# LordLiang/DrawingSpinUp

Measured on NVIDIA H100. Metric: stylized frames/sec @512x512 (stage1+stage2), higher is better.
Workload: dtype fp16x3 (split fp16 hi+lo operands, fp32 accumulate)

## Files before the change

drawingspinup_b200/csrc/conv_wgmma.cu:

```cuda
#include "conv_device.cuh"

namespace dsu {

namespace {

__host__ __device__ inline uint32_t acc_pitch(int cout) { return static_cast<uint32_t>(cout) + 4; }

__host__ __device__ inline uint32_t par_bytes(int cout) { return (7 * cout + 4) * 4; }

__host__ __device__ inline int ric_halo_rows(int up) { return (kTileH >> up) + 2; }
__host__ __device__ inline int ric_halo_cols(int up) { return (kTileW >> up) + 2; }
constexpr uint32_t kStenBytes = kTileM * 8 * 8;

__host__ __device__ constexpr int halo_rows(int cout) { return cout <= 64 ? 16 : 8; }

constexpr int kRicRegMaxCout = 128;

__host__ __device__ constexpr bool register_a(ConvMode mode, int cout) {
    return mode == ConvMode::Halo || (mode == ConvMode::RicHalo && cout <= kRicRegMaxCout);
}

__host__ __device__ constexpr int ric_ctas_per_sm(ConvMode mode, int cout) {
    return mode == ConvMode::RicHalo && cout <= 64 ? 2 : 1;
}

struct SmemLayout {
    uint32_t stage_bytes;
    uint32_t halo;
    uint32_t halo_bytes;
    uint32_t aux;
    uint32_t par;
    uint32_t total;
};

__host__ __device__ inline SmemLayout smem_layout(ConvMode mode, int cout, int ksize, int up) {
    const bool halo = mode == ConvMode::Halo, ric_halo = mode == ConvMode::RicHalo;
    const int rows = halo ? halo_rows(cout) : kTileH;
    SmemLayout L;
    L.stage_bytes = (register_a(mode, cout) ? 0u : static_cast<uint32_t>(kABytes)) + static_cast<uint32_t>(cout) * 128u;
    L.halo = kStages * L.stage_bytes;
    L.halo_bytes = halo       ? static_cast<uint32_t>((rows + ksize - 1) * (kTileW + ksize - 1)) * 128u
                   : ric_halo ? static_cast<uint32_t>(ric_halo_rows(up) * ric_halo_cols(up)) * 128u : 0u;
    L.aux = L.halo + 2 * L.halo_bytes;
    const uint32_t main_end = L.aux + (halo ? 16u : ric_halo ? kStenBytes : 0u);
    const uint32_t staged = static_cast<uint32_t>(rows * kTileW) * acc_pitch(cout) * 4u;
    L.par = ((main_end > staged ? main_end : staged) + 15u) & ~15u;
    L.total = L.par + par_bytes(cout);
    return L;
}

__device__ __forceinline__ constexpr int ric_r0(int m) { return (m >= 2 && m <= 5) ? 0 : 1; }
__device__ __forceinline__ constexpr int ric_c0(int m) { return (m >= 4) ? 0 : 1; }

__device__ __forceinline__ void produce_tap(const ConvParams& p, int q, uint32_t a, int tid, int n, int ty0, int tx0) {
    const int j = tid & 7;
    const int prow = tid >> 3;
    const Slot sl = p.slots[q * 8 + j];
    const Seg sg = p.seg[sl.seg];
    const __half* sbase = sg.ptr + sl.choff;
    const uint32_t dst0 = a + static_cast<uint32_t>(prow) * 128u + (static_cast<uint32_t>(j ^ (prow & 7)) << 4);
    const size_t frame_in = static_cast<size_t>(n) * p.Hin * p.Win;
    const int ox = tx0 + (prow & 15), oy0 = ty0 + (prow >> 4);
    const int vx = ox * p.stride + sl.dx;
    const bool okx = sl.valid && static_cast<unsigned>(vx) < static_cast<unsigned>(p.Wv);
#pragma unroll
    for (int i = 0; i < 4; ++i) {
        const int vy = (oy0 + 2 * i) * p.stride + sl.dy;
        const bool ok = okx && static_cast<unsigned>(vy) < static_cast<unsigned>(p.Hv);
        const size_t pix = frame_in + static_cast<size_t>(vy >> p.up) * p.Win + (vx >> p.up);
        cp_async16(dst0 + i * 4096u, ok ? sbase + pix * sg.pitch : sbase, ok ? 16u : 0u);
    }
}

template <bool kExact>
struct RicItems {
    static constexpr int kSlots = kExact ? 4 : 8, kRowsPer = kExact ? 2 : 4, kRowStep = kTileM / kRowsPer;
};

struct RicWeightsH { __half2 w00, w01, w10, w11; };
struct RicWeightsF { float w0, w1, w2, w3; };

__device__ __forceinline__ __half2 h2_of(uint32_t v) { return *reinterpret_cast<const __half2*>(&v); }

__device__ __forceinline__ RicWeightsH ric_weights(uint2 wv) {
    const __half2 wa = h2_of(wv.x), wb = h2_of(wv.y);
    return {__low2half2(wa), __high2half2(wa), __low2half2(wb), __high2half2(wb)};
}
__device__ __forceinline__ RicWeightsF ric_weights(float2 l) {
    const float hy = 1.0f - l.x, hx = 1.0f - l.y;
    return {__fmul_rn(hy, hx), __fmul_rn(hy, l.y), __fmul_rn(l.x, hx), __fmul_rn(l.x, l.y)};
}
__device__ __forceinline__ uint32_t ric_blend(const RicWeightsH& w, uint32_t n00, uint32_t n01, uint32_t n10, uint32_t n11) {
    const __half2 o = __hfma2(w.w11, h2_of(n11), __hfma2(w.w10, h2_of(n10), __hfma2(w.w01, h2_of(n01), __hmul2(w.w00, h2_of(n00)))));
    return *reinterpret_cast<const uint32_t*>(&o);
}
__device__ __forceinline__ float ric_blend(const RicWeightsF& w, float v00, float v01, float v10, float v11) {
    return __fmaf_rn(w.w3, v11, __fmaf_rn(w.w2, v10, __fmaf_rn(w.w1, v01, __fmul_rn(w.w0, v00))));
}

template <bool kExact, typename Entry, typename Fetch>
__device__ __forceinline__ void ric_item(bool centre, const Entry& entry, const Fetch& fetch, uint32_t row, int d, uint32_t swz) {
    if constexpr (!kExact) {
        uint4 out;
        if (centre) {
            out = fetch(0, 0, 0);
        } else {
            const RicWeightsH w = ric_weights(entry());
            const uint4 n00 = fetch(0, 0, 0), n01 = fetch(0, 1, 0), n10 = fetch(1, 0, 0), n11 = fetch(1, 1, 0);
            out = make_uint4(ric_blend(w, n00.x, n01.x, n10.x, n11.x), ric_blend(w, n00.y, n01.y, n10.y, n11.y),
                             ric_blend(w, n00.z, n01.z, n10.z, n11.z), ric_blend(w, n00.w, n01.w, n10.w, n11.w));
        }
        st_shared_v4(row + ((static_cast<uint32_t>(d) ^ swz) << 4), out);
    } else {
        auto load8 = [&](int cy, int cx, float* v) {
            const uint4 lo = fetch(cy, cx, 0), hi = fetch(cy, cx, 1);
            v[0] = __uint_as_float(lo.x); v[1] = __uint_as_float(lo.y); v[2] = __uint_as_float(lo.z); v[3] = __uint_as_float(lo.w);
            v[4] = __uint_as_float(hi.x); v[5] = __uint_as_float(hi.y); v[6] = __uint_as_float(hi.z); v[7] = __uint_as_float(hi.w);
        };
        float f[8];
        if (centre) {
            load8(0, 0, f);
        } else {
            const RicWeightsF w = ric_weights(entry());
            float v00[8], v01[8], v10[8], v11[8];
            load8(0, 0, v00); load8(0, 1, v01); load8(1, 0, v10); load8(1, 1, v11);
#pragma unroll
            for (int c = 0; c < 8; ++c) f[c] = ric_blend(w, v00[c], v01[c], v10[c], v11[c]);
        }
        uint4 hi, lo;
        split8(f, hi, lo);
        st_shared_v4(row + ((static_cast<uint32_t>(d) ^ swz) << 4), hi);
        st_shared_v4(row + ((static_cast<uint32_t>(d + 4) ^ swz) << 4), lo);
    }
}

template <bool kExact>
__device__ __forceinline__ void produce_ric(const ConvParams& p, int q, uint32_t a, int tid, int n, int ty0, int tx0) {
    using It = RicItems<kExact>;
    const int blk = q / 9, t = q - 9 * blk;
    const int kq = t < 4 ? t : t - 1;
    const size_t frame_in = static_cast<size_t>(n) * p.Hin * p.Win;
    const int d = tid % It::kSlots, prow = tid / It::kSlots;
    const Slot sl = p.slots[blk * 8 + d];
    const Seg sg = p.seg[sl.seg];
    constexpr size_t kEsz = kExact ? sizeof(float) : sizeof(__half);
    const uint8_t* src = reinterpret_cast<const uint8_t*>(sg.ptr) + sl.choff * kEsz;
    const size_t pitch = static_cast<size_t>(sg.pitch) * kEsz;
#pragma unroll
    for (int i = 0; i < It::kRowsPer; ++i) {
        const int r = prow + It::kRowStep * i;
        const int oy = ty0 + (r >> 4), ox = tx0 + (r & 15);
        const bool live = sl.valid && oy < p.Hout && ox < p.Wout;
        const size_t e = live ? static_cast<size_t>(oy) * p.Wout + ox : 0;
        int dy0 = 0, dx0 = 0, m = 0;
        if (t != 4) {
            m = (kq + __ldg(p.ric_oct + e)) & 7;
            dy0 = ric_r0(m) - 1; dx0 = ric_c0(m) - 1;
        }
        auto fetch = [&](int cy, int cx, int h) {
            const int vy = oy + dy0 + cy, vx = ox + dx0 + cx;
            const bool ok = live && static_cast<unsigned>(vy) < static_cast<unsigned>(p.Hv) && static_cast<unsigned>(vx) < static_cast<unsigned>(p.Wv);
            const size_t pix = ok ? frame_in + static_cast<size_t>(vy >> p.up) * p.Win + (vx >> p.up) : 0;
            return ldg128_if(src + pix * pitch + 16 * h, ok);
        };
        auto entry = [&]() {
            if constexpr (kExact) return live ? __ldg(p.ric_lyx + e * 8 + m) : make_float2(0.0f, 0.0f);
            else return live ? __ldg(p.ric_wh + e * 8 + m) : make_uint2(0u, 0u);
        };
        ric_item<kExact>(t == 4, entry, fetch, a + static_cast<uint32_t>(r) * 128u, d, static_cast<uint32_t>(r & 7));
    }
}

struct RicTile {
    uint32_t halo, halo_bytes;
    uint32_t sten;
    uint32_t oct;
};

template <bool kExact>
__device__ __forceinline__ void stage_ric_stencil(const ConvParams& p, uint32_t sten, int tid, int ty0, int tx0) {
    const uint8_t* table = kExact ? reinterpret_cast<const uint8_t*>(p.ric_lyx) : reinterpret_cast<const uint8_t*>(p.ric_wh);
    for (int i = tid; i < kTileM * 8; i += kThreads) {
        const int r = i >> 3, m = i & 7;
        const int oy = ty0 + (r >> 4), ox = tx0 + (r & 15);
        const bool ok = oy < p.Hout && ox < p.Wout;
        const size_t e = ok ? static_cast<size_t>(oy) * p.Wout + ox : 0;
        cp_async8(sten + static_cast<uint32_t>(m * kTileM + r) * 8u, table + (e * 8 + m) * 8, ok ? 8u : 0u);
    }
}

__device__ __forceinline__ uint32_t ric_oct(const ConvParams& p, int r, int ty0, int tx0) {
    const int oy = ty0 + (r >> 4), ox = tx0 + (r & 15);
    return (oy < p.Hout && ox < p.Wout) ? static_cast<uint32_t>(__ldg(p.ric_oct + static_cast<size_t>(oy) * p.Wout + ox)) : 0u;
}

template <bool kExact>
__device__ __forceinline__ uint32_t load_ric_stencil(const ConvParams& p, uint32_t sten, int tid, int ty0, int tx0) {
    using It = RicItems<kExact>;
    stage_ric_stencil<kExact>(p, sten, tid, ty0, tx0);
    uint32_t oct = 0;
#pragma unroll
    for (int i = 0; i < It::kRowsPer; ++i) oct |= ric_oct(p, tid / It::kSlots + It::kRowStep * i, ty0, tx0) << (8 * i);
    return oct;
}

template <bool kExact>
__device__ __forceinline__ void load_ric_halo(const ConvParams& p, int blk, uint32_t halo, int tid, int n, int ty0, int tx0) {
    const int hw = ric_halo_cols(p.up), npix = ric_halo_rows(p.up) * hw;
    const int y0 = (ty0 >> p.up) - 1, x0 = (tx0 >> p.up) - 1;
    const int s = tid & 7;
    const Slot sl = p.slots[blk * 8 + (kExact ? s >> 1 : s)];
    const Seg sg = p.seg[sl.seg];
    constexpr size_t kEsz = kExact ? sizeof(float) : sizeof(__half);
    const uint8_t* sbase = reinterpret_cast<const uint8_t*>(sg.ptr) + (sl.choff + (kExact ? 4 * (s & 1) : 0)) * kEsz;
    const size_t pitch = static_cast<size_t>(sg.pitch) * kEsz;
    const size_t frame_in = static_cast<size_t>(n) * p.Hin * p.Win;
    for (int pix = tid >> 3; pix < npix; pix += kThreads / 8) {
        const int hy = pix / hw, hx = pix - hy * hw;
        const int y = y0 + hy, x = x0 + hx;
        const bool ok = sl.valid && static_cast<unsigned>(y) < static_cast<unsigned>(p.Hin) && static_cast<unsigned>(x) < static_cast<unsigned>(p.Win);
        const uint8_t* src = ok ? sbase + (frame_in + static_cast<size_t>(y) * p.Win + x) * pitch : sbase;
        cp_async16(halo + static_cast<uint32_t>(pix) * 128u + (static_cast<uint32_t>(s ^ (pix & 7)) << 4), src, ok ? 16u : 0u);
    }
}

template <bool kExact>
__device__ __forceinline__ void produce_ric_halo(const ConvParams& p, int q, uint32_t a, int tid, int ty0, int tx0, const RicTile& rt) {
    using It = RicItems<kExact>;
    const int blk = q / 9, t = q - 9 * blk;
    const int kq = t < 4 ? t : t - 1;
    const int d = tid % It::kSlots, prow = tid / It::kSlots;
    const bool valid = p.slots[blk * 8 + d].valid;
    const uint32_t halo = rt.halo + static_cast<uint32_t>(blk & 1) * rt.halo_bytes;
    const int hw = ric_halo_cols(p.up), y0 = (ty0 >> p.up) - 1, x0 = (tx0 >> p.up) - 1;
#pragma unroll
    for (int i = 0; i < It::kRowsPer; ++i) {
        const int r = prow + It::kRowStep * i;
        const int oy = ty0 + (r >> 4), ox = tx0 + (r & 15);
        const bool live = valid && oy < p.Hout && ox < p.Wout;
        int dy0 = 0, dx0 = 0, m = 0;
        if (t != 4) {
            m = (kq + (rt.oct >> (8 * i))) & 7;
            dy0 = ric_r0(m) - 1; dx0 = ric_c0(m) - 1;
        }
        auto fetch = [&](int cy, int cx, int h) {
            const int hp = (((oy + dy0 + cy) >> p.up) - y0) * hw + ((ox + dx0 + cx) >> p.up) - x0;
            const uint32_t s = kExact ? static_cast<uint32_t>(2 * d + h) : static_cast<uint32_t>(d);
            const uint4 v = ld_shared_v4(halo + static_cast<uint32_t>(hp) * 128u + ((s ^ static_cast<uint32_t>(hp & 7)) << 4));
            return live ? v : make_uint4(0u, 0u, 0u, 0u);
        };
        auto entry = [&]() {
            const uint2 raw = ld_shared_v2(rt.sten + static_cast<uint32_t>(m * kTileM + r) * 8u);
            if constexpr (kExact) return make_float2(__uint_as_float(raw.x), __uint_as_float(raw.y));
            else return raw;
        };
        ric_item<kExact>(t == 4, entry, fetch, a + static_cast<uint32_t>(r) * 128u, d, static_cast<uint32_t>(r & 7));
    }
}

struct RicLane {
    int r;
    int oy, ox;
    uint32_t live;
    uint32_t oct;
    int ax;
    int aslot;
};

__device__ __forceinline__ RicLane ric_lane(const ConvParams& p, int tid, int ty0, int tx0) {
    const int wg = tid >> 7, w = (tid >> 5) & 3, l = tid & 31;
    RicLane ln;
    ln.r = 64 * wg + 16 * w + (l >> 2);
    ln.oy = ty0 + (ln.r >> 4);
    ln.ox = tx0 + (ln.r & 15);
    ln.live = (ln.oy < p.Hout && ln.ox < p.Wout ? 1u : 0u) | (ln.oy < p.Hout && ln.ox + 8 < p.Wout ? 2u : 0u);
    const int ra = (ln.r & ~15) + (l & 7) + 8 * ((l >> 3) & 1);
    ln.ax = tx0 + (ra & 15);
    ln.aslot = l >> 4;
    ln.oct = ric_oct(p, ln.r, ty0, tx0) | ric_oct(p, ln.r + 8, ty0, tx0) << 8 | ric_oct(p, ra, ty0, tx0) << 16;
    return ln;
}

template <bool kExact>
__device__ __forceinline__ void build_ric_a(const ConvParams& p, int q, uint32_t halo, uint32_t sten, const RicLane& ln,
                                            int lane, int ty0, int tx0, uint32_t (*a)[4]) {
    const int t = q % 9, kq = t < 4 ? t : t - 1;
    const int hw = ric_halo_cols(p.up), y0 = (ty0 >> p.up) - 1, x0 = (tx0 >> p.up) - 1;
    auto hpix = [&](int vy, int vx) { return ((vy >> p.up) - y0) * hw + (vx >> p.up) - x0; };
    auto sector = [&](int j, int& dy0, int& dx0) {
        const int m = (kq + (ln.oct >> (8 * j))) & 7;
        dy0 = ric_r0(m) - 1; dx0 = ric_c0(m) - 1;
        return m;
    };
    if constexpr (!kExact) {
        auto slot = [&](int hp, int k) { return halo + static_cast<uint32_t>(hp) * 128u + ((static_cast<uint32_t>(2 * k + ln.aslot) ^ static_cast<uint32_t>(hp & 7)) << 4); };
        if (t == 4) {
            const int hp = hpix(ln.oy, ln.ax);
#pragma unroll
            for (int k = 0; k < 4; ++k) ldsm_x4(a[k], slot(hp, k));
        } else {
            int dy0, dx0;
            sector(2, dy0, dx0);
            const int vy = ln.oy + dy0, vx = ln.ax + dx0;
            const int h00 = hpix(vy, vx), h01 = hpix(vy, vx + 1), h10 = hpix(vy + 1, vx), h11 = hpix(vy + 1, vx + 1);
            RicWeightsH w[2];
#pragma unroll
            for (int j = 0; j < 2; ++j) w[j] = ric_weights(ld_shared_v2(sten + static_cast<uint32_t>(sector(j, dy0, dx0) * kTileM + ln.r + 8 * j) * 8u));
#pragma unroll
            for (int k = 0; k < 4; ++k) {
                uint32_t n00[4], n01[4], n10[4], n11[4];
                ldsm_x4(n00, slot(h00, k)); ldsm_x4(n01, slot(h01, k)); ldsm_x4(n10, slot(h10, k)); ldsm_x4(n11, slot(h11, k));
#pragma unroll
                for (int i = 0; i < 4; ++i) a[k][i] = ric_blend(w[i & 1], n00[i], n01[i], n10[i], n11[i]);
            }
        }
#pragma unroll
        for (int k = 0; k < 4; ++k)
#pragma unroll
            for (int i = 0; i < 4; ++i)
                if (!((ln.live >> (i & 1)) & 1)) a[k][i] = 0u;
    } else {
        const uint32_t th = static_cast<uint32_t>((lane & 3) >> 1), tb = static_cast<uint32_t>(lane & 1) * 8u;
        auto ld = [&](int hp, int g) {
            const uint32_t s = 2u * g + th;
            const uint2 v = ld_shared_v2(halo + static_cast<uint32_t>(hp) * 128u + ((s ^ static_cast<uint32_t>(hp & 7)) << 4) + tb);
            return make_float2(__uint_as_float(v.x), __uint_as_float(v.y));
        };
        auto put = [&](int j, int g, float2 f) {
            if (!((ln.live >> j) & 1)) f = make_float2(0.0f, 0.0f);
            uint32_t hi, lo;
            split2(f.x, f.y, hi, lo);
            a[g >> 1][j + 2 * (g & 1)] = hi;
            a[2 + (g >> 1)][j + 2 * (g & 1)] = lo;
        };
        if (t == 4) {
            float2 v[2][4];
#pragma unroll
            for (int j = 0; j < 2; ++j) {
                const int hp = hpix(ln.oy, ln.ox + 8 * j);
#pragma unroll
                for (int g = 0; g < 4; ++g) v[j][g] = ld(hp, g);
            }
#pragma unroll
            for (int j = 0; j < 2; ++j)
#pragma unroll
                for (int g = 0; g < 4; ++g) put(j, g, v[j][g]);
        } else {
#pragma unroll
            for (int j = 0; j < 2; ++j) {
                int dy0, dx0;
                const uint2 raw = ld_shared_v2(sten + static_cast<uint32_t>(sector(j, dy0, dx0) * kTileM + ln.r + 8 * j) * 8u);
                const int vy = ln.oy + dy0, vx = ln.ox + 8 * j + dx0;
                const int h00 = hpix(vy, vx), h01 = hpix(vy, vx + 1), h10 = hpix(vy + 1, vx), h11 = hpix(vy + 1, vx + 1);
                float2 v00[4], v01[4], v10[4], v11[4];
#pragma unroll
                for (int g = 0; g < 4; ++g) { v00[g] = ld(h00, g); v01[g] = ld(h01, g); v10[g] = ld(h10, g); v11[g] = ld(h11, g); }
                const RicWeightsF w = ric_weights(make_float2(__uint_as_float(raw.x), __uint_as_float(raw.y)));
#pragma unroll
                for (int g = 0; g < 4; ++g)
                    put(j, g, make_float2(ric_blend(w, v00[g].x, v01[g].x, v10[g].x, v11[g].x),
                                          ric_blend(w, v00[g].y, v01[g].y, v10[g].y, v11[g].y)));
            }
        }
    }
}

__device__ __forceinline__ void produce_b(const ConvParams& p, int q, uint32_t dst, int tid) {
    const uint8_t* src = p.wpack + static_cast<size_t>(q) * p.b_bytes;
    for (int i = tid; i < p.b_bytes / 16; i += kThreads) cp_async16(dst + 16u * i, src + 16 * i, 16u);
}

template <ConvMode kMode, bool kExact>
__device__ __forceinline__ void produce(const ConvParams& p, int q, uint32_t stage, int tid, int n, int ty0, int tx0, const RicTile& rt) {
    if constexpr (kMode == ConvMode::Tap) {
        produce_tap(p, q, stage, tid, n, ty0, tx0);
    } else if constexpr (kMode == ConvMode::Ric) {
        produce_ric<kExact>(p, q, stage, tid, n, ty0, tx0);
    } else {
        const int blk = q / 9;
        if (q == 9 * blk && blk + 1 < p.nblocks)
            load_ric_halo<kExact>(p, blk + 1, rt.halo + static_cast<uint32_t>((blk + 1) & 1) * rt.halo_bytes, tid, n, ty0, tx0);
        produce_ric_halo<kExact>(p, q, stage, tid, ty0, tx0, rt);
    }
    produce_b(p, q, stage + kABytes, tid);
}

template <int NC, int PN>
__device__ __forceinline__ void mma_chunk(float* acc, uint64_t da, uint64_t db, uint32_t km, uint32_t km2) {
    constexpr uint64_t kPieceStep = PN * 128 / 16;
    auto step = [&](int ka, int kb) {
#pragma unroll
        for (int j = 0; j < NC / PN; ++j) Wgmma<PN>::mma(acc + j * (PN / 2), da + 2 * ka, db + 2 * kb + j * kPieceStep);
    };
    if (km2) {
#pragma unroll
        for (int k = 0; k < 4; ++k)
            if ((km >> k) & 1) step(k, k & 1);
#pragma unroll
        for (int k = 0; k < 2; ++k)
            if ((km2 >> k) & 1) step(k, 2 + k);
    } else {
#pragma unroll
        for (int k = 0; k < 4; ++k)
            if ((km >> k) & 1) step(k, k);
    }
}

template <int NC, int PN, int MB, bool kExact>
__device__ __forceinline__ void mma_chunk_rs(float (*acc)[NC / 2], const uint32_t (*a)[4][4], uint64_t db) {
    constexpr uint64_t kPieceStep = PN * 128 / 16;
    auto step = [&](int ka, int kb) {
#pragma unroll
        for (int mb = 0; mb < MB; ++mb)
#pragma unroll
            for (int j = 0; j < NC / PN; ++j) Wgmma<PN>::mma_rs(acc[mb] + j * (PN / 2), a[mb][ka], db + 2 * kb + j * kPieceStep);
    };
#pragma unroll
    for (int k = 0; k < 4; ++k) step(k, kExact ? (k & 1) : k);
    if constexpr (kExact) {
#pragma unroll
        for (int k = 0; k < 2; ++k) step(k, 2 + k);
    }
}

template <int kRows>
__device__ __forceinline__ void load_halo(const ConvParams& p, int blk, uint32_t halo, int tid, int n, int ty0, int tx0) {
    const int hw = kTileW + p.ksize - 1, npix = (kRows + p.ksize - 1) * hw;
    const int s = tid & 7;
    const Slot sl = p.hslots[blk * 8 + s];
    const Seg sg = p.seg[sl.seg];
    const __half* sbase = sg.ptr + sl.choff;
    const size_t frame_in = static_cast<size_t>(n) * p.Hin * p.Win;
    for (int pix = tid >> 3; pix < npix; pix += kThreads / 8) {
        const int hy = pix / hw, hx = pix - hy * hw;
        const int y = ty0 - p.pad_y + hy, x = tx0 - p.pad_x + hx;
        const bool ok = sl.valid && static_cast<unsigned>(y) < static_cast<unsigned>(p.Hin) && static_cast<unsigned>(x) < static_cast<unsigned>(p.Win);
        const __half* src = ok ? sbase + (frame_in + static_cast<size_t>(y) * p.Win + x) * sg.pitch : sbase;
        cp_async16(halo + static_cast<uint32_t>(pix) * 128u + (static_cast<uint32_t>(s ^ (pix & 7)) << 4), src, ok ? 16u : 0u);
    }
}

template <int MB>
__device__ __forceinline__ void load_a(const ConvParams& p, int q, uint32_t halo, uint32_t zero, const int* pb, int lane,
                                       uint32_t (*a)[4][4]) {
    const int hw = kTileW + p.ksize - 1;
    const uint2* slots = reinterpret_cast<const uint2*>(p.slots) + q * 8 + (lane >> 4);
#pragma unroll
    for (int k = 0; k < 4; ++k) {
        const uint2 raw = __ldg(slots + 2 * k);
        Slot sl;
        memcpy(&sl, &raw, sizeof(sl));
        const int shift = (sl.dy + p.pad_y) * hw + sl.dx + p.pad_x;
#pragma unroll
        for (int mb = 0; mb < MB; ++mb) {
            const int pix = pb[mb] + shift;
            const uint32_t addr = sl.valid ? halo + static_cast<uint32_t>(pix) * 128u + (static_cast<uint32_t>(sl.hslot ^ (pix & 7)) << 4) : zero;
            ldsm_x4(a[mb][k], addr);
        }
    }
}

template <int NC, int MB>
__device__ __forceinline__ void store_tile(const ConvParams& p, uint8_t* smem, const float* s_par, float (*acc)[NC / 2],
                                           int tid, int n, int ty0, int tx0) {
    constexpr int kM = 128 * MB;
    float* staged = reinterpret_cast<float*>(smem);
    {
        const int wg = tid >> 7, w = (tid >> 5) & 3, l = tid & 31;
#pragma unroll
        for (int mb = 0; mb < MB; ++mb) {
            const int r0 = wg * (kM / 2) + mb * 64 + 16 * w + (l >> 2), c0 = 2 * (l & 3);
#pragma unroll
            for (int i = 0; i < NC / 2; i += 2) {
                const int r = r0 + 8 * ((i >> 1) & 1), c = c0 + 8 * (i >> 2);
                *reinterpret_cast<float2*>(staged + r * acc_pitch(NC) + c) = make_float2(acc[mb][i], acc[mb][i + 1]);
            }
        }
    }
    __syncthreads();
#pragma unroll
    for (int i = 0; i < MB; ++i) {
        const int r = (tid & 127) + 128 * i;
        const float* row = staged + r * acc_pitch(NC);
        if (p.sub) epilogue_row<true>(p, s_par, row, n, ty0 + (r >> 4), tx0 + (r & 15), tid >> 7);
        else epilogue_row<false>(p, s_par, row, n, ty0 + (r >> 4), tx0 + (r & 15), tid >> 7);
    }
}

}

template <int NC, int PN, ConvMode kMode, bool kExact>
__global__ void __launch_bounds__(kThreads, 1)
conv_wgmma_kernel(const __grid_constant__ ConvParams p) {
    static_assert(!register_a(kMode, NC), "conv_wgmma_kernel: shared-memory A modes only");
    extern __shared__ uint8_t smem_raw[];
    const uint32_t raw_u32 = smem_u32(smem_raw);
    const uint32_t base = (raw_u32 + 1023u) & ~1023u;
    uint8_t* smem = smem_raw + (base - raw_u32);
    const SmemLayout L = smem_layout(kMode, NC, p.ksize, p.up);
    float* s_par = reinterpret_cast<float*>(smem + L.par);

    const int tid = threadIdx.x;
    const int wg = tid >> 7;
    const int n = blockIdx.z;
    const int ty0 = blockIdx.y * kTileH;
    const int tx0 = blockIdx.x * kTileW;
    const int nq = p.nchunks;
    const int tail_from = kMode != ConvMode::Tap ? (p.nblocks - 1) * 9 : nq - 1;

    load_epilogue_params(p, s_par, tid, kThreads);

    float acc[1][NC / 2];
#pragma unroll
    for (int i = 0; i < NC / 2; ++i) acc[0][i] = 0.0f;

    RicTile rt{base + L.halo, L.halo_bytes, base + L.aux, 0u};
    if constexpr (kMode == ConvMode::RicHalo) {
        rt.oct = load_ric_stencil<kExact>(p, rt.sten, tid, ty0, tx0);
        load_ric_halo<kExact>(p, 0, rt.halo, tid, n, ty0, tx0);
        cp_async_commit();
        cp_async_wait<0>();
        __syncthreads();
    }
#pragma unroll
    for (int s = 0; s < kStages - 2; ++s) {
        if (s < nq) produce<kMode, kExact>(p, s, base + s * L.stage_bytes, tid, n, ty0, tx0, rt);
        cp_async_commit();
    }
    for (int q = 0; q < nq; ++q) {
        cp_async_wait<kStages - 3>();
        fence_proxy_async_smem();
        __syncthreads();
        const uint32_t stage = base + (q % kStages) * L.stage_bytes;
        const uint64_t da = wgmma_desc_sw128(stage + wg * (kABytes / 2), 1024), db = wgmma_desc_sw128(stage + kABytes, 1024);
        const bool tail = q >= tail_from;
        wgmma_fence();
        mma_chunk<NC, PN>(acc[0], da, db, tail ? p.kmask_last : p.kmask_full, tail ? p.kmask2_last : p.kmask2_full);
        wgmma_commit();
        wgmma_wait<1>();
        if (q + kStages - 2 < nq) produce<kMode, kExact>(p, q + kStages - 2, base + ((q + kStages - 2) % kStages) * L.stage_bytes, tid, n, ty0, tx0, rt);
        cp_async_commit();
    }
    wgmma_wait<0>();
    cp_async_wait<0>();
    __syncthreads();
    store_tile<NC, 1>(p, smem, s_par, acc, tid, n, ty0, tx0);
}

template <int NC, int PN, ConvMode kMode, bool kExact>
__global__ void __launch_bounds__(kThreads, ric_ctas_per_sm(kMode, NC))
conv_halo_kernel(const __grid_constant__ ConvParams p) {
    constexpr bool kRic = kMode == ConvMode::RicHalo;
    static_assert(register_a(kMode, NC), "conv_halo_kernel: Halo, or RicHalo up to kRicRegMaxCout channels");
    constexpr int kRows = kRic ? kTileH : halo_rows(NC), kM = kRows * kTileW, MB = kM / 128;
    extern __shared__ uint8_t smem_raw[];
    const uint32_t raw_u32 = smem_u32(smem_raw);
    const uint32_t base = (raw_u32 + 1023u) & ~1023u;
    uint8_t* smem = smem_raw + (base - raw_u32);
    const SmemLayout L = smem_layout(kMode, NC, p.ksize, p.up);
    float* s_par = reinterpret_cast<float*>(smem + L.par);
    const uint32_t aux = base + L.aux;

    const int tid = threadIdx.x;
    const int wg = tid >> 7, warp = (tid >> 5) & 3, lane = tid & 31;
    const int n = blockIdx.z;
    const int ty0 = blockIdx.y * kRows;
    const int tx0 = blockIdx.x * kTileW;
    const int nq = p.nchunks, kk = kRic ? 9 : p.ksize * p.ksize;
    const int hw = kTileW + p.ksize - 1;

    load_epilogue_params(p, s_par, tid, kThreads);
    if (!kRic && tid < 4) reinterpret_cast<uint32_t*>(smem + L.aux)[tid] = 0u;

    int pb[MB];
#pragma unroll
    for (int mb = 0; mb < MB; ++mb) {
        const int r = wg * (kM / 2) + mb * 64 + warp * 16 + (lane & 15);
        pb[mb] = (r >> 4) * hw + (r & 15);
    }
    RicLane ln{};
    if constexpr (kRic) ln = ric_lane(p, tid, ty0, tx0);
    float acc[MB][NC / 2];
#pragma unroll
    for (int mb = 0; mb < MB; ++mb)
#pragma unroll
        for (int i = 0; i < NC / 2; ++i) acc[mb][i] = 0.0f;
    constexpr bool kOneBuf = ric_ctas_per_sm(kMode, NC) > 1;
    uint32_t a[2][MB][4][4];

    auto halo_buf = [&](int blk) { return base + L.halo + static_cast<uint32_t>(blk & 1) * L.halo_bytes; };
    auto load_block = [&](int blk) {
        if constexpr (kRic) load_ric_halo<kExact>(p, blk, halo_buf(blk), tid, n, ty0, tx0);
        else load_halo<kRows>(p, blk, halo_buf(blk), tid, n, ty0, tx0);
    };
    auto load_frags = [&](int q, uint32_t (*dst)[4][4]) {
        if constexpr (kRic) build_ric_a<kExact>(p, q, halo_buf(q / kk), aux, ln, lane, ty0, tx0, dst[0]);
        else load_a<MB>(p, q, halo_buf(q / kk), aux, pb, lane, dst);
    };

    if constexpr (kRic) stage_ric_stencil<kExact>(p, aux, tid, ty0, tx0);
    load_block(0);
    produce_b(p, 0, base, tid);
    cp_async_commit();
    if (nq > 1) produce_b(p, 1, base + L.stage_bytes, tid);
    cp_async_commit();
    cp_async_wait<1>();
    __syncthreads();
    load_frags(0, a[0]);

    auto step = [&](int q, const uint32_t (*cur)[4][4], uint32_t (*nxt)[4][4]) {
        cp_async_wait<kStages - 3>();
        fence_proxy_async_smem();
        __syncthreads();
        const uint64_t db = wgmma_desc_sw128(base + (q % kStages) * L.stage_bytes, 1024);
        wgmma_fence();
        mma_chunk_rs<NC, PN, MB, kExact>(acc, cur, db);
        wgmma_commit();
        if constexpr (kOneBuf) wgmma_wait<0>();
        else wgmma_wait<1>();
        if (q + 1 < nq) load_frags(q + 1, nxt);
        if (q + 2 < nq) produce_b(p, q + 2, base + ((q + 2) % kStages) * L.stage_bytes, tid);
        const int blk = q / kk;
        if (q == blk * kk && blk + 1 < p.nblocks) load_block(blk + 1);
        cp_async_commit();
    };
    for (int q = 0; q < nq; q += 2) {
        step(q, a[0], a[kOneBuf ? 0 : 1]);
        if (q + 1 < nq) step(q + 1, a[kOneBuf ? 0 : 1], a[0]);
    }
    wgmma_wait<0>();
    cp_async_wait<0>();
    __syncthreads();
    store_tile<NC, MB>(p, smem, s_par, acc, tid, n, ty0, tx0);
}

size_t conv_smem_bytes(ConvMode mode, int cout, int ksize, int up) { return smem_layout(mode, cout, ksize, up).total + 1024; }

namespace {

template <ConvMode kMode, bool kExact, int NC, int PN>
cudaError_t launch_one(const ConvParams& p, cudaStream_t stream) {
    constexpr int kRows = kMode == ConvMode::Halo ? halo_rows(NC) : kTileH;
    void (*kernel)(ConvParams);
    if constexpr (register_a(kMode, NC)) kernel = conv_halo_kernel<NC, PN, kMode, kExact>;
    else kernel = conv_wgmma_kernel<NC, PN, kMode, kExact>;
    static bool attr_set[64] = {};
    int dev = 0;
    cudaError_t e = cudaGetDevice(&dev);
    if (e == cudaSuccess && !(dev < 64 && attr_set[dev])) {
        e = cudaFuncSetAttribute(kernel, cudaFuncAttributeMaxDynamicSharedMemorySize, 227 * 1024);
        if (e == cudaSuccess && ric_ctas_per_sm(kMode, NC) > 1)
            e = cudaFuncSetAttribute(kernel, cudaFuncAttributePreferredSharedMemoryCarveout, cudaSharedmemCarveoutMaxShared);
        if (e == cudaSuccess && dev < 64) attr_set[dev] = true;
    }
    if (e != cudaSuccess) return e;
    dim3 grid((p.Wout + kTileW - 1) / kTileW, (p.Hout + kRows - 1) / kRows, p.B);
    kernel<<<grid, kThreads, conv_smem_bytes(kMode, NC, p.ksize, p.up), stream>>>(p);
    return cudaGetLastError();
}

template <ConvMode kMode, bool kExact>
cudaError_t launch_mode(const ConvParams& p, cudaStream_t stream) {
    switch (p.Cout) {
        case 32: return launch_one<kMode, kExact, 32, 32>(p, stream);
        case 64: return launch_one<kMode, kExact, 64, 64>(p, stream);
        case 96: return launch_one<kMode, kExact, 96, 32>(p, stream);
        case 128: return p.n128 ? launch_one<kMode, kExact, 128, 128>(p, stream) : launch_one<kMode, kExact, 128, 64>(p, stream);
        default: break;
    }
    if constexpr (!kExact) {
        switch (p.Cout) {
            case 160: return launch_one<kMode, kExact, 160, 32>(p, stream);
            case 192: return launch_one<kMode, kExact, 192, 64>(p, stream);
            case 224: return launch_one<kMode, kExact, 224, 32>(p, stream);
            case 256: return p.n128 ? launch_one<kMode, kExact, 256, 128>(p, stream) : launch_one<kMode, kExact, 256, 64>(p, stream);
            default: break;
        }
    }
    return cudaErrorInvalidConfiguration;
}

}

cudaError_t launch_conv(const ConvParams& p, cudaStream_t stream) {
    if (conv_smem_bytes(p.mode, p.Cout, p.ksize, p.up) > 227 * 1024 || p.b_bytes != p.Cout * 128) return cudaErrorInvalidConfiguration;
    switch (p.mode) {
        case ConvMode::Tap: return launch_mode<ConvMode::Tap, false>(p, stream);
        case ConvMode::Ric: return p.exact ? launch_mode<ConvMode::Ric, true>(p, stream) : launch_mode<ConvMode::Ric, false>(p, stream);
        case ConvMode::RicHalo:
            return p.exact ? launch_mode<ConvMode::RicHalo, true>(p, stream) : launch_mode<ConvMode::RicHalo, false>(p, stream);
        case ConvMode::Halo: return p.exact ? launch_mode<ConvMode::Halo, true>(p, stream) : launch_mode<ConvMode::Halo, false>(p, stream);
    }
    return cudaErrorInvalidConfiguration;
}

}
```

drawingspinup_b200/csrc/ptx.cuh:

```cuda
#pragma once
#include <cuda_fp16.h>
#include <stdint.h>

namespace dsu {

__device__ __forceinline__ uint32_t smem_u32(const void* p) {
    return static_cast<uint32_t>(__cvta_generic_to_shared(p));
}

__device__ __forceinline__ void cp_async16(uint32_t dst, const void* src, uint32_t src_bytes) {
    asm volatile("cp.async.cg.shared.global [%0], [%1], 16, %2;" ::"r"(dst), "l"(src), "r"(src_bytes) : "memory");
}
__device__ __forceinline__ void cp_async8(uint32_t dst, const void* src, uint32_t src_bytes) {
    asm volatile("cp.async.ca.shared.global [%0], [%1], 8, %2;" ::"r"(dst), "l"(src), "r"(src_bytes) : "memory");
}
__device__ __forceinline__ void cp_async_commit() { asm volatile("cp.async.commit_group;" ::: "memory"); }
template <int N>
__device__ __forceinline__ void cp_async_wait() { asm volatile("cp.async.wait_group %0;" ::"n"(N) : "memory"); }

__device__ __forceinline__ uint4 ld_shared_v4(uint32_t addr) {
    uint4 v;
    asm volatile("ld.shared.v4.u32 {%0, %1, %2, %3}, [%4];" : "=r"(v.x), "=r"(v.y), "=r"(v.z), "=r"(v.w) : "r"(addr) : "memory");
    return v;
}
__device__ __forceinline__ uint2 ld_shared_v2(uint32_t addr) {
    uint2 v;
    asm volatile("ld.shared.v2.u32 {%0, %1}, [%2];" : "=r"(v.x), "=r"(v.y) : "r"(addr) : "memory");
    return v;
}
__device__ __forceinline__ void st_shared_v4(uint32_t addr, const uint4& v) {
    asm volatile("st.shared.v4.u32 [%0], {%1, %2, %3, %4};" ::"r"(addr), "r"(v.x), "r"(v.y), "r"(v.z), "r"(v.w) : "memory");
}

__device__ __forceinline__ void ldsm_x4(uint32_t* r, uint32_t addr) {
    asm volatile("ldmatrix.sync.aligned.m8n8.x4.shared.b16 {%0, %1, %2, %3}, [%4];"
                 : "=r"(r[0]), "=r"(r[1]), "=r"(r[2]), "=r"(r[3]) : "r"(addr) : "memory");
}

__device__ __forceinline__ void fence_proxy_async_smem() {
    asm volatile("fence.proxy.async.shared::cta;" ::: "memory");
}

__device__ __forceinline__ uint4 ldg128_if(const void* ptr, bool ok) {
    uint4 v;
    asm("{\n\t.reg .pred p;\n\tsetp.ne.u32 p, %5, 0;\n\tmov.u32 %0, 0;\n\tmov.u32 %1, 0;\n\tmov.u32 %2, 0;\n\tmov.u32 %3, 0;\n\t"
        "@p ld.global.nc.v4.u32 {%0, %1, %2, %3}, [%4];\n\t}"
        : "=r"(v.x), "=r"(v.y), "=r"(v.z), "=r"(v.w)
        : "l"(ptr), "r"(static_cast<uint32_t>(ok)));
    return v;
}

__device__ __forceinline__ uint64_t wgmma_desc_sw128(uint32_t smem_addr, uint32_t sbo_bytes) {
    uint64_t d = 0;
    d |= static_cast<uint64_t>((smem_addr >> 4) & 0x3FFFu);
    d |= static_cast<uint64_t>(1) << 16;
    d |= static_cast<uint64_t>((sbo_bytes >> 4) & 0x3FFFu) << 32;
    d |= static_cast<uint64_t>(1) << 62;
    return d;
}

__device__ __forceinline__ void wgmma_fence() { asm volatile("wgmma.fence.sync.aligned;" ::: "memory"); }
__device__ __forceinline__ void wgmma_commit() { asm volatile("wgmma.commit_group.sync.aligned;" ::: "memory"); }
template <int N>
__device__ __forceinline__ void wgmma_wait() { asm volatile("wgmma.wait_group.sync.aligned %0;" ::"n"(N) : "memory"); }

template <int N>
struct Wgmma;

template <>
struct Wgmma<32> {
    __device__ __forceinline__ static void mma(float* d, uint64_t a, uint64_t b) {
        asm volatile(
            "{\n\t.reg .pred p;\n\tsetp.ne.b32 p, 1, 0;\n\t"
            "wgmma.mma_async.sync.aligned.m64n32k16.f32.f16.f16 "
            "{%0, %1, %2, %3, %4, %5, %6, %7, %8, %9, %10, %11, %12, %13, %14, %15}, %16, %17, p, 1, 1, 0, 0;\n\t}"
            : "+f"(d[0]), "+f"(d[1]), "+f"(d[2]), "+f"(d[3]), "+f"(d[4]), "+f"(d[5]), "+f"(d[6]), "+f"(d[7]),
              "+f"(d[8]), "+f"(d[9]), "+f"(d[10]), "+f"(d[11]), "+f"(d[12]), "+f"(d[13]), "+f"(d[14]), "+f"(d[15])
            : "l"(a), "l"(b));
    }
    __device__ __forceinline__ static void mma_rs(float* d, const uint32_t* a, uint64_t b) {
        asm volatile(
            "{\n\t.reg .pred p;\n\tsetp.ne.b32 p, 1, 0;\n\t"
            "wgmma.mma_async.sync.aligned.m64n32k16.f32.f16.f16 "
            "{%0, %1, %2, %3, %4, %5, %6, %7, %8, %9, %10, %11, %12, %13, %14, %15}, {%16, %17, %18, %19}, %20, p, 1, 1, 0;\n\t}"
            : "+f"(d[0]), "+f"(d[1]), "+f"(d[2]), "+f"(d[3]), "+f"(d[4]), "+f"(d[5]), "+f"(d[6]), "+f"(d[7]),
              "+f"(d[8]), "+f"(d[9]), "+f"(d[10]), "+f"(d[11]), "+f"(d[12]), "+f"(d[13]), "+f"(d[14]), "+f"(d[15])
            : "r"(a[0]), "r"(a[1]), "r"(a[2]), "r"(a[3]), "l"(b));
    }
};

template <>
struct Wgmma<64> {
    __device__ __forceinline__ static void mma(float* d, uint64_t a, uint64_t b) {
        asm volatile(
            "{\n\t.reg .pred p;\n\tsetp.ne.b32 p, 1, 0;\n\t"
            "wgmma.mma_async.sync.aligned.m64n64k16.f32.f16.f16 "
            "{%0, %1, %2, %3, %4, %5, %6, %7, %8, %9, %10, %11, %12, %13, %14, %15, "
            "%16, %17, %18, %19, %20, %21, %22, %23, %24, %25, %26, %27, %28, %29, %30, %31}, %32, %33, p, 1, 1, 0, 0;\n\t}"
            : "+f"(d[0]), "+f"(d[1]), "+f"(d[2]), "+f"(d[3]), "+f"(d[4]), "+f"(d[5]), "+f"(d[6]), "+f"(d[7]),
              "+f"(d[8]), "+f"(d[9]), "+f"(d[10]), "+f"(d[11]), "+f"(d[12]), "+f"(d[13]), "+f"(d[14]), "+f"(d[15]),
              "+f"(d[16]), "+f"(d[17]), "+f"(d[18]), "+f"(d[19]), "+f"(d[20]), "+f"(d[21]), "+f"(d[22]), "+f"(d[23]),
              "+f"(d[24]), "+f"(d[25]), "+f"(d[26]), "+f"(d[27]), "+f"(d[28]), "+f"(d[29]), "+f"(d[30]), "+f"(d[31])
            : "l"(a), "l"(b));
    }
    __device__ __forceinline__ static void mma_rs(float* d, const uint32_t* a, uint64_t b) {
        asm volatile(
            "{\n\t.reg .pred p;\n\tsetp.ne.b32 p, 1, 0;\n\t"
            "wgmma.mma_async.sync.aligned.m64n64k16.f32.f16.f16 "
            "{%0, %1, %2, %3, %4, %5, %6, %7, %8, %9, %10, %11, %12, %13, %14, %15, %16, %17, %18, %19, %20, %21, %22, %23, %24, %25, %26, %27, %28, %29, %30, %31}, {%32, %33, %34, %35}, %36, p, 1, 1, 0;\n\t}"
            : "+f"(d[0]), "+f"(d[1]), "+f"(d[2]), "+f"(d[3]), "+f"(d[4]), "+f"(d[5]), "+f"(d[6]), "+f"(d[7]),
              "+f"(d[8]), "+f"(d[9]), "+f"(d[10]), "+f"(d[11]), "+f"(d[12]), "+f"(d[13]), "+f"(d[14]), "+f"(d[15]),
              "+f"(d[16]), "+f"(d[17]), "+f"(d[18]), "+f"(d[19]), "+f"(d[20]), "+f"(d[21]), "+f"(d[22]), "+f"(d[23]),
              "+f"(d[24]), "+f"(d[25]), "+f"(d[26]), "+f"(d[27]), "+f"(d[28]), "+f"(d[29]), "+f"(d[30]), "+f"(d[31])
            : "r"(a[0]), "r"(a[1]), "r"(a[2]), "r"(a[3]), "l"(b));
    }
};

template <>
struct Wgmma<128> {
    __device__ __forceinline__ static void mma(float* d, uint64_t a, uint64_t b) {
        asm volatile(
            "{\n\t.reg .pred p;\n\tsetp.ne.b32 p, 1, 0;\n\t"
            "wgmma.mma_async.sync.aligned.m64n128k16.f32.f16.f16 "
            "{%0, %1, %2, %3, %4, %5, %6, %7, %8, %9, %10, %11, %12, %13, %14, %15, %16, %17, %18, %19, %20, %21, %22, %23, %24, %25, %26, %27, %28, %29, %30, %31, %32, %33, %34, %35, %36, %37, %38, %39, %40, %41, %42, %43, %44, %45, %46, %47, %48, %49, %50, %51, %52, %53, %54, %55, %56, %57, %58, %59, %60, %61, %62, %63}, %64, %65, p, 1, 1, 0, 0;\n\t}"
            : "+f"(d[0]), "+f"(d[1]), "+f"(d[2]), "+f"(d[3]), "+f"(d[4]), "+f"(d[5]), "+f"(d[6]), "+f"(d[7]),
              "+f"(d[8]), "+f"(d[9]), "+f"(d[10]), "+f"(d[11]), "+f"(d[12]), "+f"(d[13]), "+f"(d[14]), "+f"(d[15]),
              "+f"(d[16]), "+f"(d[17]), "+f"(d[18]), "+f"(d[19]), "+f"(d[20]), "+f"(d[21]), "+f"(d[22]), "+f"(d[23]),
              "+f"(d[24]), "+f"(d[25]), "+f"(d[26]), "+f"(d[27]), "+f"(d[28]), "+f"(d[29]), "+f"(d[30]), "+f"(d[31]),
              "+f"(d[32]), "+f"(d[33]), "+f"(d[34]), "+f"(d[35]), "+f"(d[36]), "+f"(d[37]), "+f"(d[38]), "+f"(d[39]),
              "+f"(d[40]), "+f"(d[41]), "+f"(d[42]), "+f"(d[43]), "+f"(d[44]), "+f"(d[45]), "+f"(d[46]), "+f"(d[47]),
              "+f"(d[48]), "+f"(d[49]), "+f"(d[50]), "+f"(d[51]), "+f"(d[52]), "+f"(d[53]), "+f"(d[54]), "+f"(d[55]),
              "+f"(d[56]), "+f"(d[57]), "+f"(d[58]), "+f"(d[59]), "+f"(d[60]), "+f"(d[61]), "+f"(d[62]), "+f"(d[63])
            : "l"(a), "l"(b));
    }
    __device__ __forceinline__ static void mma_rs(float* d, const uint32_t* a, uint64_t b) {
        asm volatile(
            "{\n\t.reg .pred p;\n\tsetp.ne.b32 p, 1, 0;\n\t"
            "wgmma.mma_async.sync.aligned.m64n128k16.f32.f16.f16 "
            "{%0, %1, %2, %3, %4, %5, %6, %7, %8, %9, %10, %11, %12, %13, %14, %15, %16, %17, %18, %19, %20, %21, %22, %23, %24, %25, %26, %27, %28, %29, %30, %31, %32, %33, %34, %35, %36, %37, %38, %39, %40, %41, %42, %43, %44, %45, %46, %47, %48, %49, %50, %51, %52, %53, %54, %55, %56, %57, %58, %59, %60, %61, %62, %63}, {%64, %65, %66, %67}, %68, p, 1, 1, 0;\n\t}"
            : "+f"(d[0]), "+f"(d[1]), "+f"(d[2]), "+f"(d[3]), "+f"(d[4]), "+f"(d[5]), "+f"(d[6]), "+f"(d[7]),
              "+f"(d[8]), "+f"(d[9]), "+f"(d[10]), "+f"(d[11]), "+f"(d[12]), "+f"(d[13]), "+f"(d[14]), "+f"(d[15]),
              "+f"(d[16]), "+f"(d[17]), "+f"(d[18]), "+f"(d[19]), "+f"(d[20]), "+f"(d[21]), "+f"(d[22]), "+f"(d[23]),
              "+f"(d[24]), "+f"(d[25]), "+f"(d[26]), "+f"(d[27]), "+f"(d[28]), "+f"(d[29]), "+f"(d[30]), "+f"(d[31]),
              "+f"(d[32]), "+f"(d[33]), "+f"(d[34]), "+f"(d[35]), "+f"(d[36]), "+f"(d[37]), "+f"(d[38]), "+f"(d[39]),
              "+f"(d[40]), "+f"(d[41]), "+f"(d[42]), "+f"(d[43]), "+f"(d[44]), "+f"(d[45]), "+f"(d[46]), "+f"(d[47]),
              "+f"(d[48]), "+f"(d[49]), "+f"(d[50]), "+f"(d[51]), "+f"(d[52]), "+f"(d[53]), "+f"(d[54]), "+f"(d[55]),
              "+f"(d[56]), "+f"(d[57]), "+f"(d[58]), "+f"(d[59]), "+f"(d[60]), "+f"(d[61]), "+f"(d[62]), "+f"(d[63])
            : "r"(a[0]), "r"(a[1]), "r"(a[2]), "r"(a[3]), "l"(b));
    }
};

}
```

Before: 128.2.

## Replace cp.async and block barriers with mbarrier ring and bulk weight copies

Replaces the register-A conv kernel's cp.async pipeline and per-step __syncthreads with an mbarrier-based producer/consumer ring. Weight chunks are fetched by a single thread with cp.async.bulk into a deeper ring, sized up to eight stages within the shared-memory limit. Halo tiles now signal full and empty through mbarriers. The aim is to remove CTA-wide barriers and deepen weight prefetch so the warpgroups can run ahead independently. It adds phase-tracking complexity and the risk of hangs or races, and the larger smem footprint may lower occupancy. The accumulators are also zeroed through a volatile asm move.

```diff
diff --git a/drawingspinup_b200/csrc/conv_wgmma.cu b/drawingspinup_b200/csrc/conv_wgmma.cu
--- a/drawingspinup_b200/csrc/conv_wgmma.cu
+++ b/drawingspinup_b200/csrc/conv_wgmma.cu
@@ -24,28 +24,43 @@
     return mode == ConvMode::RicHalo && cout <= 64 ? 2 : 1;
 }
 
+constexpr int kMaxRing = 8;
+__host__ __device__ constexpr int ring_cap(ConvMode mode) { return mode == ConvMode::Halo ? kMaxRing : kStages; }
+
 struct SmemLayout {
+    uint32_t stages;
     uint32_t stage_bytes;
     uint32_t halo;
     uint32_t halo_bytes;
     uint32_t aux;
     uint32_t par;
+    uint32_t bars;
     uint32_t total;
 };
 
-__host__ __device__ inline SmemLayout smem_layout(ConvMode mode, int cout, int ksize, int up) {
+__host__ __device__ inline SmemLayout smem_layout_at(ConvMode mode, int cout, int ksize, int up, int stages) {
     const bool halo = mode == ConvMode::Halo, ric_halo = mode == ConvMode::RicHalo;
     const int rows = halo ? halo_rows(cout) : kTileH;
     SmemLayout L;
+    L.stages = static_cast<uint32_t>(stages);
     L.stage_bytes = (register_a(mode, cout) ? 0u : static_cast<uint32_t>(kABytes)) + static_cast<uint32_t>(cout) * 128u;
-    L.halo = kStages * L.stage_bytes;
+    L.halo = L.stages * L.stage_bytes;
     L.halo_bytes = halo       ? static_cast<uint32_t>((rows + ksize - 1) * (kTileW + ksize - 1)) * 128u
                    : ric_halo ? static_cast<uint32_t>(ric_halo_rows(up) * ric_halo_cols(up)) * 128u : 0u;
     L.aux = L.halo + 2 * L.halo_bytes;
     const uint32_t main_end = L.aux + (halo ? 16u : ric_halo ? kStenBytes : 0u);
     const uint32_t staged = static_cast<uint32_t>(rows * kTileW) * acc_pitch(cout) * 4u;
     L.par = ((main_end > staged ? main_end : staged) + 15u) & ~15u;
-    L.total = L.par + par_bytes(cout);
+    L.bars = L.par + par_bytes(cout);
+    L.total = L.bars + (register_a(mode, cout) ? (2 * L.stages + 4) * 8u : 0u);
+    return L;
+}
+
+__host__ __device__ inline SmemLayout smem_layout(ConvMode mode, int cout, int ksize, int up) {
+    if (!register_a(mode, cout)) return smem_layout_at(mode, cout, ksize, up, kStages);
+    SmemLayout L = smem_layout_at(mode, cout, ksize, up, ring_cap(mode));
+    for (int s = ring_cap(mode) - 1; s >= kStages && L.total + 1024u > 227u * 1024u; --s)
+        L = smem_layout_at(mode, cout, ksize, up, s);
     return L;
 }
 
@@ -584,52 +599,99 @@
 #pragma unroll
     for (int mb = 0; mb < MB; ++mb)
 #pragma unroll
-        for (int i = 0; i < NC / 2; ++i) acc[mb][i] = 0.0f;
+        for (int i = 0; i < NC / 2; ++i) acc[mb][i] = pinned_zero();
     constexpr bool kOneBuf = ric_ctas_per_sm(kMode, NC) > 1;
     uint32_t a[2][MB][4][4];
+
+    const int S = static_cast<int>(L.stages);
+    const uint32_t bars = base + L.bars;
+    auto full_bar = [&](int s) { return bars + 8u * static_cast<uint32_t>(s); };
+    auto empty_bar = [&](int s) { return bars + 8u * static_cast<uint32_t>(S + s); };
+    auto hfull_bar = [&](int blk) { return bars + 8u * static_cast<uint32_t>(2 * S + (blk & 1)); };
+    auto hempty_bar = [&](int blk) { return bars + 8u * static_cast<uint32_t>(2 * S + 2 + (blk & 1)); };
+    if (tid == 0) {
+        for (int s = 0; s < S; ++s) {
+            mbar_init(full_bar(s), 1);
+            mbar_init(empty_bar(s), 2);
+        }
+        for (int i = 0; i < 2; ++i) {
+            mbar_init(hfull_bar(i), kThreads);
+            mbar_init(hempty_bar(i), kThreads / 32);
+        }
+        fence_mbar_init();
+    }
+    __syncthreads();
 
     auto halo_buf = [&](int blk) { return base + L.halo + static_cast<uint32_t>(blk & 1) * L.halo_bytes; };
     auto load_block = [&](int blk) {
         if constexpr (kRic) load_ric_halo<kExact>(p, blk, halo_buf(blk), tid, n, ty0, tx0);
         else load_halo<kRows>(p, blk, halo_buf(blk), tid, n, ty0, tx0);
+        cp_async_mbar_arrive(hfull_bar(blk));
     };
-    auto load_frags = [&](int q, uint32_t (*dst)[4][4]) {
-        if constexpr (kRic) build_ric_a<kExact>(p, q, halo_buf(q / kk), aux, ln, lane, ty0, tx0, dst[0]);
-        else load_a<MB>(p, q, halo_buf(q / kk), aux, pb, lane, dst);
+    auto load_frags = [&](int q, int b, uint32_t (*dst)[4][4]) {
+        if constexpr (kRic) build_ric_a<kExact>(p, q, halo_buf(b), aux, ln, lane, ty0, tx0, dst[0]);
+        else load_a<MB>(p, q, halo_buf(b), aux, pb, lane, dst);
+    };
+    auto produce_w = [&](int c, int s) {
+        mbar_arrive_expect_tx(full_bar(s), static_cast<uint32_t>(p.b_bytes));
+        bulk_copy_g2s(base + static_cast<uint32_t>(s) * L.stage_bytes, p.wpack + static_cast<size_t>(c) * p.b_bytes,
+                      static_cast<uint32_t>(p.b_bytes), full_bar(s));
     };
 
     if constexpr (kRic) stage_ric_stencil<kExact>(p, aux, tid, ty0, tx0);
     load_block(0);
-    produce_b(p, 0, base, tid);
-    cp_async_commit();
-    if (nq > 1) produce_b(p, 1, base + L.stage_bytes, tid);
-    cp_async_commit();
-    cp_async_wait<1>();
-    __syncthreads();
-    load_frags(0, a[0]);
-
+    if (tid == 0)
+        for (int c = 0; c < S - 2 && c < nq; ++c) produce_w(c, c);
+    mbar_wait(hfull_bar(0), 0);
+    load_frags(0, 0, a[0]);
+
+    int qs = 0, cblk = 0, cqt = 0;
+    uint32_t qph = 0;
     auto step = [&](int q, const uint32_t (*cur)[4][4], uint32_t (*nxt)[4][4]) {
-        cp_async_wait<kStages - 3>();
-        fence_proxy_async_smem();
-        __syncthreads();
-        const uint64_t db = wgmma_desc_sw128(base + (q % kStages) * L.stage_bytes, 1024);
+        mbar_wait(full_bar(qs), qph);
+        const uint64_t db = wgmma_desc_sw128(base + static_cast<uint32_t>(qs) * L.stage_bytes, 1024);
         wgmma_fence();
         mma_chunk_rs<NC, PN, MB, kExact>(acc, cur, db);
         wgmma_commit();
-        if constexpr (kOneBuf) wgmma_wait<0>();
-        else wgmma_wait<1>();
-        if (q + 1 < nq) load_frags(q + 1, nxt);
-        if (q + 2 < nq) produce_b(p, q + 2, base + ((q + 2) % kStages) * L.stage_bytes, tid);
-        const int blk = q / kk;
-        if (q == blk * kk && blk + 1 < p.nblocks) load_block(blk + 1);
-        cp_async_commit();
+        if constexpr (kOneBuf) {
+            wgmma_wait<0>();
+            if ((tid & 127) == 0) mbar_arrive(empty_bar(qs));
+        } else {
+            wgmma_wait<1>();
+            if (q > 0 && (tid & 127) == 0) mbar_arrive(empty_bar(qs > 0 ? qs - 1 : S - 1));
+        }
+        if (tid == 0 && q + S - 2 < nq) {
+            const int ps = qs >= 2 ? qs - 2 : qs + S - 2;
+            if (q >= 2) mbar_wait(empty_bar(ps), qs >= 2 ? qph : qph ^ 1u);
+            produce_w(q + S - 2, ps);
+        }
+        const int blk = kRic ? q / 9 : cblk, qt = kRic ? q - 9 * blk : cqt;
+        const bool next_blk = qt + 1 == kk;
+        const int nb = next_blk ? blk + 1 : blk, nt = next_blk ? 0 : qt + 1;
+        if (q + 1 < nq) {
+            if (next_blk) mbar_wait(hfull_bar(nb), static_cast<uint32_t>(nb >> 1) & 1u);
+            load_frags(q + 1, nb, nxt);
+            if (nt + 1 == kk || q + 2 == nq) {
+                __syncwarp();
+                if (lane == 0) mbar_arrive(hempty_bar(nb));
+            }
+        }
+        if (qt == 0 && blk + 1 < p.nblocks) {
+            if (blk >= 1) mbar_wait(hempty_bar(blk + 1), (static_cast<uint32_t>((blk + 1) >> 1) & 1u) ^ 1u);
+            load_block(blk + 1);
+        }
+        cblk = nb;
+        cqt = nt;
+        if (++qs == S) {
+            qs = 0;
+            qph ^= 1u;
+        }
     };
     for (int q = 0; q < nq; q += 2) {
         step(q, a[0], a[kOneBuf ? 0 : 1]);
         if (q + 1 < nq) step(q + 1, a[kOneBuf ? 0 : 1], a[0]);
     }
     wgmma_wait<0>();
-    cp_async_wait<0>();
     __syncthreads();
     store_tile<NC, MB>(p, smem, s_par, acc, tid, n, ty0, tx0);
 }
diff --git a/drawingspinup_b200/csrc/ptx.cuh b/drawingspinup_b200/csrc/ptx.cuh
--- a/drawingspinup_b200/csrc/ptx.cuh
+++ b/drawingspinup_b200/csrc/ptx.cuh
@@ -41,6 +41,31 @@
     asm volatile("fence.proxy.async.shared::cta;" ::: "memory");
 }
 
+__device__ __forceinline__ void mbar_init(uint32_t bar, uint32_t count) {
+    asm volatile("mbarrier.init.shared::cta.b64 [%0], %1;" ::"r"(bar), "r"(count) : "memory");
+}
+__device__ __forceinline__ void fence_mbar_init() { asm volatile("fence.mbarrier_init.release.cluster;" ::: "memory"); }
+__device__ __forceinline__ void mbar_arrive(uint32_t bar) {
+    asm volatile("mbarrier.arrive.release.cta.shared::cta.b64 _, [%0];" ::"r"(bar) : "memory");
+}
+__device__ __forceinline__ void mbar_arrive_expect_tx(uint32_t bar, uint32_t bytes) {
+    asm volatile("mbarrier.arrive.expect_tx.release.cta.shared::cta.b64 _, [%0], %1;" ::"r"(bar), "r"(bytes) : "memory");
+}
+__device__ __forceinline__ void mbar_wait(uint32_t bar, uint32_t parity) {
+    asm volatile(
+        "{\n\t.reg .pred done;\n"
+        "wait_%=:\n\t"
+        "mbarrier.try_wait.parity.acquire.cta.shared::cta.b64 done, [%0], %1;\n\t"
+        "@!done bra wait_%=;\n\t}" ::"r"(bar), "r"(parity) : "memory");
+}
+__device__ __forceinline__ void cp_async_mbar_arrive(uint32_t bar) {
+    asm volatile("cp.async.mbarrier.arrive.noinc.shared::cta.b64 [%0];" ::"r"(bar) : "memory");
+}
+__device__ __forceinline__ void bulk_copy_g2s(uint32_t dst, const void* src, uint32_t bytes, uint32_t bar) {
+    asm volatile("cp.async.bulk.shared::cluster.global.mbarrier::complete_tx::bytes [%0], [%1], %2, [%3];"
+                 ::"r"(dst), "l"(src), "r"(bytes), "r"(bar) : "memory");
+}
+
 __device__ __forceinline__ uint4 ldg128_if(const void* ptr, bool ok) {
     uint4 v;
     asm("{\n\t.reg .pred p;\n\tsetp.ne.u32 p, %5, 0;\n\tmov.u32 %0, 0;\n\tmov.u32 %1, 0;\n\tmov.u32 %2, 0;\n\tmov.u32 %3, 0;\n\t"
@@ -48,6 +73,12 @@
         : "=r"(v.x), "=r"(v.y), "=r"(v.z), "=r"(v.w)
         : "l"(ptr), "r"(static_cast<uint32_t>(ok)));
     return v;
+}
+
+__device__ __forceinline__ float pinned_zero() {
+    float z;
+    asm volatile("mov.b32 %0, 0;" : "=f"(z));
+    return z;
 }
 
 __device__ __forceinline__ uint64_t wgmma_desc_sw128(uint32_t smem_addr, uint32_t sbo_bytes) {
```

Result: faster. 144.0 (median of 6 runs) (+12.3%).
